# shreyasren/GPU-DualGradient-MPC

Hardware: AMD Instinct MI355X
Metric: GPAD iterations/s (instance-iterations, solve to eps=1e-4) (higher is better)
Workload: dtype f32

## Files before the change

### gpu-dualgradient-mpc_amd/csrc/gpad_compact.hip

```cpp
#include <hip/hip_runtime.h>

#include "gpad_internal.h"

namespace gpad {

constexpr int kSortMax = 8192;
constexpr int kSortBins = 4096;
__device__ __forceinline__ int block_scan_1024(int* part, int tid, int v) {
    const int lane = tid & 63, w = tid >> 6;
    int x = v;
#pragma unroll
    for (int off = 1; off < 64; off <<= 1) {
        const int y = __shfl_up(x, off);
        if (lane >= off) x += y;
    }
    if (lane == 63) part[w] = x;
    __syncthreads();
    int wb = 0;
    for (int i = 0; i < w; ++i) wb += part[i];
    __syncthreads();
    return wb + x - v;
}

constexpr int kCompactMaxPanels = 8192;
constexpr int kCompactU = 8;
__global__ __launch_bounds__(1024) void phase_compact_kernel(const int* __restrict__ seg_cnt,
                                                             const int* __restrict__ seg_idx, const int* count_prev,
                                                             int batch, int fin_prev, int* idx, int* count_out,
                                                             const int* pred, int fin_cur) {
    __shared__ int hist[kSortBins];
    __shared__ int ids[kSortMax];
    __shared__ int part[1024];
    __shared__ int pbase[kCompactMaxPanels];
    __shared__ int pcnt[kCompactMaxPanels];
    __shared__ int total_l;
    const int tid = threadIdx.x;
    const int pmax = (batch + 15) / 16;
    const int per = (pmax + 1023) / 1024;
    const int p0 = tid * per < pmax ? tid * per : pmax, p1 = p0 + per < pmax ? p0 + per : pmax;
    constexpr int kPer = 8;
    int cl[kPer];
#pragma unroll
    for (int u = 0; u < kPer; ++u) cl[u] = (per <= kPer && p0 + u < p1) ? seg_cnt[p0 + u] : 0;
    const int prev = count_prev ? *count_prev : batch;
    if (count_prev && prev <= fin_prev) {
        if (tid == 0) *count_out = 0;
        return;
    }
    const int panels = (prev + 15) / 16;
    const bool lds_bases = panels <= kCompactMaxPanels;
    const int q1 = p1 < panels ? p1 : panels;
    int sum = 0;
    if (per <= kPer) {
#pragma unroll
        for (int u = 0; u < kPer; ++u) {
            if (p0 + u < q1) {
                if (lds_bases) pcnt[p0 + u] = cl[u];
                sum += cl[u];
            }
        }
    } else {
        for (int p = p0; p < q1; ++p) {
            const int c = seg_cnt[p];
            if (lds_bases) pcnt[p] = c;
            sum += c;
        }
    }
    int base = block_scan_1024(part, tid, sum);
    if (tid == 1023) total_l = base + sum;
    if (lds_bases) {
        for (int p = p0; p < q1; ++p) {
            const int c = pcnt[p];
            pbase[p] = c ? base : -1;
            base += c;
        }
    }
    __syncthreads();
    const int count = total_l;
    const bool sort = pred && count > 1 && count <= fin_cur && count <= kSortMax;
    int* dst = sort ? ids : idx;
    if (lds_bases) {
        for (int i0 = tid; i0 < 16 * panels; i0 += 1024 * kCompactU) {
            int v[kCompactU], at[kCompactU];
#pragma unroll
            for (int u = 0; u < kCompactU; ++u) {
                const int i = i0 + 1024 * u;
                at[u] = -1;
                v[u] = 0;
                if (i < 16 * panels) {
                    const int p = i >> 4, r = i & 15, b = pbase[p];
                    if (b >= 0 && r < pcnt[p]) {
                        at[u] = b + r;
                        v[u] = seg_idx[i];
                    }
                }
            }
#pragma unroll
            for (int u = 0; u < kCompactU; ++u)
                if (at[u] >= 0) dst[at[u]] = v[u];
        }
    } else {
        for (int p = p0; p < q1; ++p) {
            const int c = seg_cnt[p];
            for (int r = 0; r < c; ++r) dst[base + r] = seg_idx[16 * p + r];
            base += c;
        }
    }
    if (tid == 0) *count_out = count;
    if (!sort) return;
    __syncthreads();
    int bn[kSortMax / 1024];
#pragma unroll
    for (int u = 0; u < kSortMax / 1024; ++u) {
        const int i = tid + 1024 * u;
        bn[u] = 0;
        if (i < count) {
            const int q = pred[ids[i]];
            const int k = q < 0 ? 0 : (q >= kSortBins ? kSortBins - 1 : q);
            bn[u] = kSortBins - 1 - k;
        }
    }
    for (int i = tid; i < kSortBins; i += 1024) hist[i] = 0;
    __syncthreads();
#pragma unroll
    for (int u = 0; u < kSortMax / 1024; ++u)
        if (tid + 1024 * u < count) atomicAdd(&hist[bn[u]], 1);
    __syncthreads();
    int local[4], hs = 0;
#pragma unroll
    for (int q = 0; q < 4; ++q) {
        local[q] = hs;
        hs += hist[4 * tid + q];
    }
    const int hb = block_scan_1024(part, tid, hs);
#pragma unroll
    for (int q = 0; q < 4; ++q) hist[4 * tid + q] = hb + local[q];
    __syncthreads();
#pragma unroll
    for (int u = 0; u < kSortMax / 1024; ++u) {
        const int i = tid + 1024 * u;
        if (i < count) idx[atomicAdd(&hist[bn[u]], 1)] = ids[i];
    }
}

hipError_t launch_phase_compact(const int* seg_cnt, const int* seg_idx, const int* count_prev, int batch,
                                int fin_prev, int* idx_out, int* count_out, const int* pred, int fin_cur,
                                hipStream_t s) {
    hipLaunchKernelGGL(phase_compact_kernel, dim3(1), dim3(1024), 0, s, seg_cnt, seg_idx, count_prev, batch,
                       fin_prev, idx_out, count_out, pred, fin_cur);
    return hipGetLastError();
}

}
```

### gpu-dualgradient-mpc_amd/csrc/gpad_host.cpp

```cpp
#include <algorithm>
#include <cmath>
#include <memory>

#include "gpad_host.h"

static thread_local std::string g_last_error;

int gpad::set_last_error(int code, const std::string& msg) {
    g_last_error = msg;
    return code;
}

int reset_status(gpad_handle_t h, double tol, double floor_scale) {
    const bool fresh = h->status.p == nullptr;
    int rc = h->status.ensure(sizeof(RunStatus));
    if (rc) return rc;
    if (fresh) HIP_TRY(hipMemsetAsync(h->status.p, 0, sizeof(RunStatus), h->stream));
    h->last_tol = tol;
    h->last_floor_scale = floor_scale;
    h->failed_run = false;
    return GPAD_OK;
}

static int fetch_status(gpad_handle_t h, RunStatus* rs, bool maxima = false) {
// ... 130 lines not shown
}

const char* gpad_last_error(void) { return g_last_error.c_str(); }

int gpad_create(gpad_handle_t* out, int device, void* stream) {
    return gpad::abi_guard("gpad_create", [&]() -> int {
        if (!out) return fail(GPAD_ERR_INVALID, "gpad_create: null handle pointer");
        *out = nullptr;
        int count = 0;
        const hipError_t e = hipGetDeviceCount(&count);
        if (e != hipSuccess) return fail(GPAD_ERR_NO_DEVICE, hip_detail("gpad_create: hipGetDeviceCount", e));
        if (count <= 0) return fail(GPAD_ERR_NO_DEVICE, "gpad_create: hipGetDeviceCount reported 0 devices");
        if (device < 0 || device >= count)
            return fail(GPAD_ERR_INVALID, "gpad_create: bad device index " + std::to_string(device) + " (" +
                                              std::to_string(count) + " visible)");
        HIP_TRY(hipSetDevice(device));
        auto h = std::make_unique<gpad_handle_s>();
        h->device = device;
        h->stream = static_cast<hipStream_t>(stream);
        {
            hipDeviceProp_t prop;
            if (hipGetDeviceProperties(&prop, device) == hipSuccess && prop.multiProcessorCount > 0)
                h->num_cus = prop.multiProcessorCount;
        }
        HIP_TRY(hipEventCreate(&h->ev0));
        HIP_TRY(hipEventCreate(&h->ev1));
        *out = h.release();
        return GPAD_OK;
    });
}

int gpad_destroy(gpad_handle_t h) {
    return gpad::abi_guard("gpad_destroy", [&]() -> int {
        if (!h) return GPAD_OK;
        (void)hipSetDevice(h->device);
        (void)hipStreamSynchronize(h->stream);
        end_classes(h);
        h->MGt.release();
        h->GLt.release();
        h->GLx.release();
        h->Hq.release();
        h->frows.release();
        h->frag64.release();
        h->hfrag64.release();
        h->q64.release();
        h->p64_order.release();
        h->frag.release();
        h->stage.release();
        h->theta.release();
        h->beta.release();
        h->work.release();
        h->counters.release();
        h->pwork.release();
        h->lipwork.release();
        h->status.release();
        h->own_plant.release();
        h->state.release();
        if (h->ev0) (void)hipEventDestroy(h->ev0);
        if (h->ev1) (void)hipEventDestroy(h->ev1);
        if (h->plan_ev) (void)hipEventDestroy(h->plan_ev);
        if (h->plan_pin) (void)hipHostFree(h->plan_pin);
        delete h;
        return GPAD_OK;
    });
}

int gpad_set_stream(gpad_handle_t h, void* stream) {
    return gpad::abi_guard("gpad_set_stream", [&]() -> int {
        if (!h) return fail(GPAD_ERR_INVALID, "gpad_set_stream: null handle");
        HIP_TRY(hipSetDevice(h->device));
        HIP_TRY(hipStreamSynchronize(h->stream));
        h->stream = static_cast<hipStream_t>(stream);
        if (h->cls) return gpad::classes_set_stream(h->cls, h->stream);
        return GPAD_OK;
    });
}

int gpad_set_option(gpad_handle_t h, int option, int value) {
    return gpad::abi_guard("gpad_set_option", [&]() -> int {
        if (!h) return fail(GPAD_ERR_INVALID, "gpad_set_option: null handle");
        const int rc = set_own_option(h, option, value);
        if (rc || !h->cls) return rc;
        HIP_TRY(hipSetDevice(h->device));
        return gpad::classes_set_option(h->cls, option, value);
    });
}

int gpad_sync(gpad_handle_t h) {
    return gpad::abi_guard("gpad_sync", [&]() -> int {
        if (!h) return fail(GPAD_ERR_INVALID, "gpad_sync: null handle");
        HIP_TRY(hipSetDevice(h->device));
        if (h->cls) return gpad::classes_sync(h->cls);
        RunStatus& rs = h->h_status;
        int rc = fetch_status(h, &rs);
        if (rc) return rc;
        HIP_TRY(hipStreamSynchronize(h->stream));
        return status_error(h, rs);
    });
}

int gpad_accumulate_iterations(gpad_handle_t h, long long* acc) {
    return gpad::abi_guard("gpad_accumulate_iterations", [&]() -> int {
        if (!h || !acc) return fail(GPAD_ERR_INVALID, "gpad_accumulate_iterations: null argument");
        if (h->cls) {
            HIP_TRY(hipSetDevice(h->device));
            return gpad::classes_accumulate(h->cls, acc);
// ... 187 lines not shown
```

### gpu-dualgradient-mpc_amd/csrc/gpad_host.h

```cpp
#pragma once

#include <hip/hip_runtime.h>

#include <cstddef>
#include <string>
#include <vector>

#include "../../include/gpad.h"
#include "gpad_abi.h"
#include "gpad_classes.h"
#include "gpad_internal.h"

inline int fail(int code, const std::string& msg) { return gpad::set_last_error(code, msg); }

inline std::string hip_detail(const std::string& what, hipError_t e) {
    return what + ": " + hipGetErrorName(e) + " (code " + std::to_string((int)e) + "): " + hipGetErrorString(e);
}

#define HIP_TRY(expr)                                                                        \
    do {                                                                                     \
        hipError_t _e = (expr);                                                              \
        if (_e != hipSuccess) {                                                              \
            return fail(_e == hipErrorOutOfMemory ? GPAD_ERR_NOMEM : GPAD_ERR_HIP,           \
                        hip_detail(#expr, _e));                                              \
// ... 48 lines not shown
    {GPAD_OPT_FLAT_WAVES, &gpad::Tuning::flat_waves, 0, 16, false},
    {GPAD_OPT_FLAT_A_LDS, &gpad::Tuning::flat_a_lds, 0, 1, false},
    {GPAD_OPT_DEBUG_DROP_HANDOFF, &gpad::Tuning::debug_drop_handoff, 0, 1, false},
    {GPAD_OPT_P64_RELAY, &gpad::Tuning::p64_no_relay, 0, 1, true},
    {GPAD_OPT_P64_REFILL, &gpad::Tuning::p64_no_refill, 0, 1, true},
    {GPAD_OPT_LOOP_ASYNC, &gpad::Tuning::loop_async, 0, 1, false},
    {GPAD_OPT_LOOP_PANEL, &gpad::Tuning::loop_panel, 0, 1, false},
};

struct RunStatus {
    int err;
    int pad;
    double part[gpad::kAbsmaxMaxBlocks];
    double acc[gpad::kAbsmaxMaxBlocks];
};

struct gpad_handle_s {
    int device = 0;
    hipStream_t stream = nullptr;
    bool ready = false;
    bool flat = false;
    int n_u = 0;
    gpad_dims_t dims{};
    double L = 1.0;
    bool scaled = false;
    int ldn = 0, ldm = 0;
    DevBuf MGt, GLt, frag, stage;
    bool frag_ok = false;
    bool keep_stage = false;
    std::vector<unsigned char> shadow;
    gpad_dims_t shadow_dims{};
    double shadow_L = 0.0;
    bool shadow_ok = false;
    DevBuf GLx;
    DevBuf Hq;
    bool hess_ok = false;
    double zbound = 0.0;
    DevBuf frows;
    DevBuf frag64;
    bool frag64_ok = false;
    int frag64_tiles = 0;
    DevBuf hfrag64;
    DevBuf q64;
    DevBuf p64_order;
    std::vector<int> p64_order_host;
    int p64_order_batch = 0;
    bool p64_order_dirty = false;
    bool last_p64 = false;
    bool hfrag64_ok = false;
    int frag_tiles = 0;
    DevBuf theta, beta;
    int sched_len = 0, sched_kind = -1, sched_dtype = -1;
    DevBuf work, counters, pwork;
    DevBuf lipwork;
    std::vector<int> h_counts;
    DevBuf status;
    RunStatus h_status;
    double last_tol = 0.0;
    double last_floor_scale = 0.0;
    hipEvent_t ev0 = nullptr, ev1 = nullptr;
    int last_kernel = 0, last_batch = 0, last_steps = 1;
    bool last_phased = false;
    int last_N = 0;
    gpad::PanelPlan plan;
    unsigned long long plan_key = 0;
    gpad::PanelPlan prior;
    bool last_prior = false;
    gpad::PanelPlan last_phases;
    int flat_vpred = 0;
    int* plan_pin = nullptr;
    size_t plan_pin_cap = 0;
    hipEvent_t plan_ev = nullptr;
    bool plan_pending = false;
    int plan_pending_N = 0, plan_pending_batch = 0;
    bool plan_pending_p64 = false;
    gpad::PlantStore own_plant;
    const gpad::PlantStore* plant = &own_plant;
    int plant_first = 0;
    bool plant_all = true;
    DevBuf state;
    int num_cus = 256;
    bool timed = false;
    gpad::Tuning tune;
    gpad::ClassBinding* cls = nullptr;
    const gpad::ClassLoop* cloop = nullptr;
    bool failed_run = false;
};

int reset_status(gpad_handle_t h, double tol, double floor_scale);
int collect_stats(gpad_handle_t h, gpad_stats_t* st);
void end_classes(gpad_handle_t h);
int no_classes(const char* fn);

int validate_dims(const gpad_dims_t* d);
void unbind_problem(gpad_handle_t h);
int ensure_schedule(gpad_handle_t h, int N, const void* theta_in, const void* beta_in);

void attach_plant(gpad_handle_t h, const gpad::PlantStore* store, int first, bool all);
bool loop_panel_shape(gpad_handle_t h, int N, double tol, int nxa);

void update_plan(gpad_handle_t h, const int* counts, int batch, int N);
void build_p64_order(gpad_handle_t h, const int* counts, int batch);
template <typename T>
void fill_solve_args(gpad_handle_t h, int N, double tol, gpad::SolveArgs<T>* a);
template <typename T>
int launch_solve(gpad_handle_t h, T* dz, T* dy, const T* dM, const T* dg, int N, double tol, bool scaled_vec,
// ... 2 lines not shown
```

### gpu-dualgradient-mpc_amd/csrc/gpad_internal.h

```cpp
#pragma once

#include <hip/hip_runtime.h>

#include <cstdint>
#include <string>

namespace gpad {

int set_last_error(int code, const std::string& msg);

struct ClassBinding;

struct Tuning {
    int phase_len = 0;
    int finish_thresh = -1;
    int plan = 1;
    int phased = 1;
    int lpt = 1;
    int panel_max_grid = 0;
    int duo_max_grid = 0;
    int flat_panel_min = -1;
    int flat_panels = 0;
    int flat_waves = 0;
    int flat_a_lds = 1;
// ... 26 lines not shown
}

template <typename T>
struct SolveArgs {
    const T* MGt;
    const T* GLt;
    long long strideA;
    long long strideB;
    const void* frag;
    int frag_tiles;
    const T* gP;
    const T* g;
    long long ld_gP, ld_g;
    double gscale;
    T* z;
    T* y;
    int n, m, ldn, ldm;
    int batch, N, check_every;
    double tol, L;
    double tol_gap;
    const T* theta;
    const T* beta;
    int* iters;
    int* conv;
    int num_cus;
    void* pwork;
    int v_begin, v_end;
    int v_pred;
    const int* idx_in;
    const int* count_in;
    int* idx_out;
    int* count_out;
    int* seg_cnt;
    int* seg_idx;
    double* gmax_part;
    int* zero_w;
    int zero_n;
    float* wc;
    float* uc;
    int fin_thresh;
    int* qctr;
    const int* pred;
    int n_u;
    int flat_staged;
    const int* order;
    const struct PanelPlan* plan;
    struct PanelPlan* used;
    const Tuning* tune;
    const T* Hq;
    long long strideHq;
    const void* hfrag64;
    int* err;
    int debug;
};

struct FarkasArgs;
template <typename T>
hipError_t launch_stream(const SolveArgs<T>& a, hipStream_t s, const FarkasArgs* fk = nullptr);
hipError_t launch_resident(const SolveArgs<float>& a, hipStream_t s, bool* supported, const FarkasArgs* fk = nullptr);
hipError_t launch_duo(const SolveArgs<float>& a, int grid, hipStream_t s);
bool resident_supported(int n, int m);
constexpr int kLoopMaxState = 64;
struct LoopArgs {
    SolveArgs<float> s;
    const float* PM;
    const float* M0;
    const float* Pg;
    const float* g0;
    const float* A;
    const float* B;
    const float* x_in;
    float* x_out;
    float* xs;
    float* us;
    double* gmax;
    int nx, nu, steps, warm;
    int per_plant;
    int ns;
    const float* S;
    int cls_K;
    const int* cls_off;
    const int* cls_start;
};
bool loop_supported(int n, int m, int nx, int nu);
int loop_blocks_per_cu(const LoopArgs& a, bool farkas = false);
hipError_t launch_loop(const LoopArgs& a, int grid, hipStream_t s, const FarkasArgs* fk = nullptr);
bool loop_panel_supported(int n, int m, int nx, int nu);
int loop_panel_grid(int n, int m, int batch, int num_cus, const Tuning* t);
hipError_t launch_loop_panel(const LoopArgs& a, int grid, hipStream_t s, const FarkasArgs* fk = nullptr);
bool panel64_supported(int n, int m);
int panel64_tiles(int n, int m);
size_t panel64_frag_bytes(int n, int m);
hipError_t launch_pack_panel64(const double* src, int rows, int cols, double scale, int T, void* dst, hipStream_t s);
hipError_t launch_panel64(const SolveArgs<double>& a, hipStream_t s);

typedef const __attribute__((address_space(4))) SolveArgs<float> KernArgs;
__device__ __forceinline__ KernArgs& kargs() {
    KernArgs* p = (KernArgs*)__builtin_amdgcn_kernarg_segment_ptr();
    asm volatile("" : "+s"(p));
    return *p;
}

template <class Args>
__device__ __forceinline__ void list_survivors(const Args& a, int P, bool park, int inst, int lane,
                                               int j) {
    const unsigned long long lv = __ballot(park && j == 0);
// ... 120 lines not shown
```

### gpu-dualgradient-mpc_amd/csrc/gpad_pairs.hip

```cpp
#include <hip/hip_runtime.h>

#include "gpad_internal.h"
#include "gpad_panel.h"

namespace gpad {

#ifdef GPAD_STAMP
#ifndef GPAD_STAMP_V0
#define GPAD_STAMP_V0 101
#endif
#ifndef GPAD_STAMP_PHASE_V
#define GPAD_STAMP_PHASE_V 100
#endif
constexpr int kStampV0 = GPAD_STAMP_V0, kStampIts = 4, kStampPts = 8;
__device__ unsigned long long g_stamps[16][kStampIts][kStampPts];
#define GPAD_STAMP_AT(P)                                      \
    do {                                                      \
        __builtin_amdgcn_sched_barrier(0);                    \
        stv[P] = __builtin_amdgcn_s_memtime();                \
        __builtin_amdgcn_sched_barrier(0);                    \
    } while (0)
#define GPAD_STAMP_FLUSH()                                                                  \
    do {                                                                                    \
        if (blockIdx.x == 0 && v >= kStampV0 && v < kStampV0 + kStampIts && lane == 0)      \
            for (int q_ = 0; q_ < kStampPts; ++q_) g_stamps[threadIdx.x >> 6][v - kStampV0][q_] = stv[q_]; \
    } while (0)
#define GPAD_STAMP_DECL unsigned long long stv[kStampPts] = {0, 0, 0, 0, 0, 0, 0, 0};
constexpr int kStampPhaseV = GPAD_STAMP_PHASE_V, kStampPhasePts = 10;
__device__ unsigned long long g_pstamps[16][kStampPhasePts];
#define GPAD_PSTAMP(P)                                                                              \
    do {                                                                                            \
        __builtin_amdgcn_sched_barrier(0);                                                          \
        if (blockIdx.x == 0 && a.v_begin == kStampPhaseV && (threadIdx.x & 63) == 0)               \
            g_pstamps[threadIdx.x >> 6][P] = __builtin_amdgcn_s_memtime();                          \
        __builtin_amdgcn_sched_barrier(0);                                                          \
    } while (0)
#define GPAD_STAMP_PTR(P) (&stv[P])
#define GPAD_PSTAMP_END(P)                  \
    do {                                    \
        if (v >= a.v_end) GPAD_PSTAMP(P);   \
    } while (0)
#else
#define GPAD_PSTAMP_END(P) \
    do {                   \
    } while (0)
#define GPAD_STAMP_AT(P) \
    do {                 \
    } while (0)
#define GPAD_STAMP_FLUSH() \
    do {                   \
    } while (0)
#define GPAD_STAMP_DECL
#define GPAD_STAMP_PTR(P) nullptr
#define GPAD_PSTAMP(P) \
    do {               \
    } while (0)
#endif

}

#include "gpad_pairs.h"

namespace gpad {

template <int T, int KQ, bool DROP = false>
__global__ __launch_bounds__(1024) void gpad_panel2_kernel(SolveArgs<float> a) {
    static_assert(T > 8 && T <= 16, "panel pairs need 8 < T <= 16");
    constexpr int D = 2 * T - 16;
    __shared__ Panel2Lds<T> L;
    const int count = a.count_in ? __builtin_amdgcn_readfirstlane(*a.count_in) : a.batch;
    if (a.count_in && count <= a.fin_thresh) return;
    const int panels = (count + 15) / 16;
    const bool pair = panels > (int)gridDim.x;
    const int w0 = __builtin_amdgcn_readfirstlane(threadIdx.x >> 6);
    const int w = pair ? ((w0 >> 1) == 4 ? w0 + 4 : ((w0 >> 1) == 6 ? w0 - 4 : w0)) : 15 - w0;
    const int items = pair ? (panels + 1) / 2 : panels;
    const bool ho = Handoff<T>::on && (KQ > 0 || (16 * (T - 1) < a.n && 16 * (T - 1) < a.m &&
                                                  (a.m + 15) / 16 == T && (a.n + 15) / 16 == T));
    if (threadIdx.x < 6) L.hflag[threadIdx.x] = 0;
    if (threadIdx.x == 0) {
        L.herr = 0;
        L.hdrop = DROP && blockIdx.x == 0;
    }
    if (threadIdx.x < 16) L.gred[threadIdx.x] = 0.0f;
    if (blockIdx.x == 0) {
        if (a.zero_w)
            for (int i = threadIdx.x; i < a.zero_n; i += blockDim.x) a.zero_w[i] = 0;
        if (a.gmax_part && a.v_begin == 0)
            for (int i = gridDim.x + threadIdx.x; i < kAbsmaxMaxBlocks; i += blockDim.x) a.gmax_part[i] = 0.0;
    }
    __syncthreads();
    if constexpr (Handoff<T>::on) {
        using H = Handoff<T>;
        if (pair) {
            if (w < D) panel2_run<T, 2, 0, 0, 0, false, KQ, DROP>(a, L, w, 0, true, items, count);
            else if (ho && w >= 14)
                panel2_run<T, 1, 1, 0, H::S, false, KQ, DROP>(a, L, T - 1, w & 1, true, items, count, HoSlots{-1, w & 1});
            else if (ho && w >= 12)
                panel2_run<T, 1, 2, H::S, 0, false, KQ, DROP>(a, L, T - 2, w & 1, true, items, count, HoSlots{w & 1, -1});
            else panel2_run<T, 1, 0, 0, 0, false, KQ, DROP>(a, L, D + ((w - D) >> 1), (w - D) & 1, true, items, count);
        } else {
            if constexpr (!H::relay) {
                if (w < T) panel2_run<T, 1, 0, 0, 0, false, 0, DROP>(a, L, w, 0, false, items, count);
                else panel2_run<T, 0, 0, 0, 0, false, 0, DROP>(a, L, 0, 0, false, items, count);
            } else if (ho && w == T - 1) panel2_run<T, 1, 2, H::R2, 0, true, 0, DROP>(a, L, w, 0, false, items, count, HoSlots{1, -1});
            else if (ho && w == T)
                panel2_run<T, 0, 3, 0, H::R1, true, 0, DROP>(a, L, T - 1, 0, false, items, count, HoSlots{-1, 0});
            else if (ho && w == T + 1)
                panel2_run<T, 0, 3, H::R1, H::R2, true, 0, DROP>(a, L, T - 1, 0, false, items, count, HoSlots{0, 1});
            else if (w < T)
                panel2_run<T, 1, 0, 0, 0, false, 0, DROP>(a, L, w, 0, false, items, count);
            else panel2_run<T, 0, 0, 0, 0, false, 0, DROP>(a, L, 0, 0, false, items, count);
        }
    } else if (pair) {
        if (w < D) panel2_run<T, 2, 0, 0, 0, false, KQ, DROP>(a, L, w, 0, true, items, count);
        else panel2_run<T, 1, 0, 0, 0, false, KQ, DROP>(a, L, D + ((w - D) >> 1), (w - D) & 1, true, items, count);
    } else {
        if (w < T) panel2_run<T, 1, 0, 0, 0, false, 0, DROP>(a, L, w, 0, false, items, count);
        else panel2_run<T, 0, 0, 0, 0, false, 0, DROP>(a, L, 0, 0, false, items, count);
    }
    if (Handoff<T>::on || a.gmax_part) {
        __syncthreads();
        if (Handoff<T>::on && threadIdx.x == 0 && L.herr) atomicOr(a.err, kDevErrHandoff);
        if (a.gmax_part && threadIdx.x == 0) {
            float g = 0.0f;
            for (int i = 0; i < 16; ++i) g = absmax_nan(g, L.gred[i]);
            a.gmax_part[blockIdx.x] = a.v_begin == 0 ? (double)g : absmax_nan(a.gmax_part[blockIdx.x], (double)g);
        }
    }
}

template <int T>
static void launch_pairs_t(const SolveArgs<float>& a, int grid, hipStream_t s) {
    if constexpr (T == 13) {
        const int kq1 = (a.m - 16 * (T - 1) + 3) / 4, kq2 = (a.n - 16 * (T - 1) + 3) / 4;
        const bool full = panel_handoff_shape(T, a.n, a.m) && kq1 == kq2;
        if (a.debug & kDebugDropHandoff) {
            if (full && kq1 == 2) hipLaunchKernelGGL((gpad_panel2_kernel<T, 2, true>), dim3(grid), dim3(1024), 0, s, a);
            else hipLaunchKernelGGL((gpad_panel2_kernel<T, 0, true>), dim3(grid), dim3(1024), 0, s, a);
            return;
        }
        if (full && kq1 == 1) { hipLaunchKernelGGL((gpad_panel2_kernel<T, 1>), dim3(grid), dim3(1024), 0, s, a); return; }
        if (full && kq1 == 2) { hipLaunchKernelGGL((gpad_panel2_kernel<T, 2>), dim3(grid), dim3(1024), 0, s, a); return; }
        if (full && kq1 == 3) { hipLaunchKernelGGL((gpad_panel2_kernel<T, 3>), dim3(grid), dim3(1024), 0, s, a); return; }
        if (full && kq1 == 4) { hipLaunchKernelGGL((gpad_panel2_kernel<T, 4>), dim3(grid), dim3(1024), 0, s, a); return; }
    }
    hipLaunchKernelGGL((gpad_panel2_kernel<T, 0>), dim3(grid), dim3(1024), 0, s, a);
}

hipError_t launch_panel_pairs(int T, const SolveArgs<float>& a, int grid, hipStream_t s) {
    switch (T) {
        case 9: launch_pairs_t<9>(a, grid, s); break;
        case 10: launch_pairs_t<10>(a, grid, s); break;
        case 11: launch_pairs_t<11>(a, grid, s); break;
        case 12: launch_pairs_t<12>(a, grid, s); break;
        case 13: launch_pairs_t<13>(a, grid, s); break;
        case 14: launch_pairs_t<14>(a, grid, s); break;
        case 15: launch_pairs_t<15>(a, grid, s); break;
        case 16: launch_pairs_t<16>(a, grid, s); break;
        default: return hipErrorInvalidValue;
    }
    return hipGetLastError();
}

#ifdef GPAD_STAMP
hipError_t read_stamps(unsigned long long* out, size_t bytes) {
    size_t b0 = bytes > sizeof(g_stamps) ? sizeof(g_stamps) : bytes;
    hipError_t e = hipMemcpyFromSymbol(out, HIP_SYMBOL(g_stamps), b0, 0, hipMemcpyDeviceToHost);
    if (e != hipSuccess || bytes <= sizeof(g_stamps)) return e;
    size_t b1 = bytes - sizeof(g_stamps);
    if (b1 > sizeof(g_pstamps)) b1 = sizeof(g_pstamps);
    return hipMemcpyFromSymbol(out + sizeof(g_stamps) / 8, HIP_SYMBOL(g_pstamps), b1, 0, hipMemcpyDeviceToHost);
}
#endif

}
```

### gpu-dualgradient-mpc_amd/csrc/gpad_phases.cpp

```cpp
#include <hip/hip_runtime.h>

#include <vector>

#include "gpad_farkas.h"
#include "gpad_internal.h"
#include "gpad_panel.h"

namespace gpad {

int panel_phase_len(int check_every, const Tuning* t) {
    int len = 4 * check_every;
    if (t && t->phase_len > 0) len = t->phase_len;
    return ((len + check_every - 1) / check_every) * check_every;
}

int panel_fin_thresh(int n, int m, int num_cus, const Tuning* t) {
    int f = resident_supported(n, m) ? 2 * num_cus : 0;
    if (t && t->finish_thresh >= 0 && f) f = t->finish_thresh;
    return f;
}

namespace {
struct PlanModel {
    int T, n, m, num_cus, grid;
// ... 161 lines not shown
    return w;
}
}

size_t panel_work_bytes(int m, int batch) { return phase_work(nullptr, m, batch).bytes; }

static hipError_t launch_panel_phase(int T, const SolveArgs<float>& a, int grid, hipStream_t s,
                                     const FarkasArgs* fk) {
    if (fk) return launch_panel_single(T, a, grid, s, fk);
    if (T == 0) {
        (void)launch_bigpanel(a, grid, s);
        return hipGetLastError();
    }
    return T > 8 ? launch_panel_pairs(T, a, grid, s) : launch_panel_single(T, a, grid, s);
}

static hipError_t launch_panel_phases(int T, SolveArgs<float> a, hipStream_t s, const FarkasArgs* fk) {
    const int panels = (a.batch + 15) / 16;
    const int resident = fk && T > 8 ? 2 * a.num_cus : panel_resident_grid(T, a.num_cus);
    int grid = panels < resident ? panels : resident;
    const Tuning tn = a.tune ? *a.tune : Tuning{};
    if (tn.panel_max_grid > 0 && tn.panel_max_grid < grid) grid = tn.panel_max_grid;
    const bool phased = a.tol > 0.0 && a.pwork != nullptr && tn.phased;
    a.fin_thresh = phased && !fk ? panel_fin_thresh(a.n, a.m, a.num_cus, &tn) : 0;
    if (!phased) {
        a.v_begin = 0;
        a.v_end = a.N;
        a.idx_in = nullptr;
        a.count_in = nullptr;
        return launch_panel_phase(T, a, grid, s, fk);
    }
    const PhaseWork w = phase_work(a.pwork, a.m, a.batch);
    a.wc = w.wc;
    a.uc = w.uc;
    a.seg_idx = w.seg_idx;
    a.seg_cnt = w.seg_cnt;
    a.idx_out = nullptr;
    a.count_out = nullptr;
    hipError_t e = hipSuccess;
    if (T > 8 && !fk) {
        a.zero_w = w.counts;
        a.zero_n = 2 * kPanelMaxPhases;
    } else if ((e = hipMemsetAsync(w.counts, 0, sizeof(int) * 2 * kPanelMaxPhases, s)) != hipSuccess) {
        return e;
    }
    const int len = panel_phase_len(a.check_every, &tn);
    const PanelPlan* plan = (a.plan && a.plan->nph > 0 && a.plan->N == a.N) ? a.plan : nullptr;
    if (a.used) {
        a.used->nph = 0;
        a.used->N = a.N;
        a.used->cost_us = plan ? plan->cost_us : 0.0;
    }
    const int fin_default = a.fin_thresh;
    int fin_prev = 0;
    int v0 = 0;
    for (int ph = 0; v0 < a.N; ++ph) {
        int plen = len;
        if (ph >= 10 && tn.phase_len <= 0) plen = len << (ph - 9 < 20 ? ph - 9 : 20);
        a.fin_thresh = fin_default;
        if (plan && ph < plan->nph) {
            plen = plan->ends[ph] - v0;
            if (ph && fin_default) a.fin_thresh = plan->fins[ph];
        }
        if (plen < 1) plen = len;
        if (ph >= kPanelMaxPhases - 1) plen = a.N;
        const int v1 = (a.N - v0 <= plen) ? a.N : v0 + plen;
        a.v_begin = v0;
        a.v_end = v1;
        a.idx_in = ph ? w.idx0 : nullptr;
        a.count_in = ph ? w.counts + ph - 1 : nullptr;
        if (ph) {
            e = launch_phase_compact(a.seg_cnt, a.seg_idx, ph >= 2 ? w.counts + ph - 2 : nullptr, a.batch, fin_prev,
                                     w.idx0, w.counts + ph - 1, (a.pred && tn.lpt) ? a.pred : nullptr, a.fin_thresh, s);
            if (e != hipSuccess) return e;
        }
        fin_prev = a.fin_thresh;
        if (a.used && ph < kPanelMaxPhases) {
            a.used->ends[ph] = v1;
            a.used->fins[ph] = ph ? a.fin_thresh : 0;
            a.used->nph = ph + 1;
        }
        if (ph && a.fin_thresh) {
            a.qctr = w.qctrs + ph;
            int g = a.fin_thresh < a.num_cus ? a.fin_thresh : a.num_cus;
            if (tn.duo_max_grid > 0 && tn.duo_max_grid < g) g = tn.duo_max_grid;
            if ((e = launch_duo(a, g, s)) != hipSuccess) return e;
        }
        if ((e = launch_panel_phase(T, a, grid, s, fk)) != hipSuccess) return e;
        a.zero_w = nullptr;
        v0 = v1;
    }
    return hipSuccess;
}

bool panel_folds_gmax(int n, int m) { return panel_tiles_for(n, m) > 8; }

hipError_t launch_panel(const SolveArgs<float>& a, hipStream_t s, bool* supported, const FarkasArgs* fk) {
    const int T = panel_tiles_for(a.n, a.m);
    if (fk && T < 1) {
        *supported = false;
        return hipSuccess;
    }
    *supported = a.frag != nullptr && a.strideA == 0 && a.strideB == 0 &&
                 (T ? a.frag_tiles == T
                    : bigpanel_supported(a.n, a.m) && a.frag_tiles == panel_tiles(a.n, a.m, a.batch));
    return *supported ? launch_panel_phases(T, a, s, fk) : hipSuccess;
}

hipError_t launch_flatpanel(const SolveArgs<float>& a0, hipStream_t s) {
    if (!flatpanel_supported(a0.n, a0.m, a0.n_u) || !a0.frag) return hipErrorInvalidValue;
    SolveArgs<float> a = a0;
    const Tuning tn = a.tune ? *a.tune : Tuning{};
    a.v_begin = 0;
    a.v_end = a.N;
    a.idx_in = nullptr;
    a.count_in = nullptr;
    const int panels = (a.batch + 15) / 16;
    const bool phased = a.tol > 0.0 && a.pwork != nullptr &&
                        (tn.phased == 2 || (tn.phased == 1 && panels >= 4 * a.num_cus));
    if (!phased) return launch_flatpanel_once(a, s);
    const PhaseWork w = phase_work(a.pwork, a.m, a.batch);
    a.wc = w.wc;
    a.uc = w.uc;
    hipError_t e = hipMemsetAsync(w.counts, 0, sizeof(int) * kPanelMaxPhases, s);
    if (e != hipSuccess) return e;
    int v0 = 0;
    for (int ph = 0; v0 < a.N; ++ph) {
        int plen = ph >= kPanelMaxPhases - 1 ? a.N : flat_phase_len(v0, a.check_every, &tn);
        if (a0.v_pred > 0 && v0 >= a0.v_pred) plen = a.N;
        const int v1 = (a.N - v0 <= plen) ? a.N : v0 + plen;
        a.v_begin = v0;
        a.v_end = v1;
        a.idx_in = ph ? ((ph & 1) ? w.idx0 : w.idx1) : nullptr;
        a.count_in = ph ? w.counts + ph - 1 : nullptr;
        a.idx_out = (ph & 1) ? w.idx1 : w.idx0;
        a.count_out = w.counts + ph;
        if ((e = launch_flatpanel_once(a, s)) != hipSuccess) return e;
        v0 = v1;
    }
// ... 5 lines not shown
```

### gpu-dualgradient-mpc_amd/csrc/gpad_run.cpp

```cpp
#include <algorithm>
#include <cmath>
#include <cstring>
#include <map>
#include <mutex>
#include <tuple>

#include "gpad_farkas.h"
#include "gpad_host.h"

using PlanShape = std::tuple<int, int, int, int, int, int, int>;
static std::mutex g_prior_mu;
static std::map<PlanShape, gpad::PanelPlan>& prior_plans() {
    static std::map<PlanShape, gpad::PanelPlan> m;
    return m;
}
static PlanShape plan_shape(gpad_handle_t h, int batch, int N) {
    return PlanShape{h->dims.n, h->dims.m, batch, h->dims.check_every, N, h->num_cus, h->tune.finish_thresh};
}
static void plan_prior_store(gpad_handle_t h, int batch, int N) {
    if (h->plan.nph <= 0) return;
    std::lock_guard<std::mutex> lk(g_prior_mu);
    auto& m = prior_plans();
    if (m.size() >= 64 && !m.count(plan_shape(h, batch, N))) m.clear();
    m[plan_shape(h, batch, N)] = h->plan;
// ... 163 lines not shown
                    if (int ro = h->p64_order.ensure(sizeof(int) * (size_t)batch)) return ro;
                    HIP_TRY(hipMemcpyAsync(h->p64_order.p, h->p64_order_host.data(), sizeof(int) * (size_t)batch,
                                           hipMemcpyHostToDevice, h->stream));
                    h->p64_order_dirty = false;
                }
                a.order = static_cast<const int*>(h->p64_order.p);
            }
            e = gpad::launch_panel64(a, h->stream);
            if (e != hipSuccess) return fail(GPAD_ERR_HIP, hip_detail("f64 panel", e));
            h->last_p64 = tol > 0.0;
            *kernel_out = GPAD_KERNEL_PANEL;
            return finish(GPAD_OK);
        }
    }
    if (a.Hq) {
        if (kernel != GPAD_KERNEL_AUTO && kernel != GPAD_KERNEL_STREAM)
            return fail(GPAD_ERR_UNSUPPORTED, "the value-function test (gpad_setup_hessian) runs on the stream kernel "
                                              "(f32) or the stream / f64 panel kernels (f64)");
        kernel = GPAD_KERNEL_STREAM;
    }
    if constexpr (sizeof(T) == sizeof(float)) {
        if (kernel == GPAD_KERNEL_STREAM && !h->flat) {
        } else if (h->flat) {
            a.n_u = h->n_u;
            const int fpm = h->tune.flat_panel_min >= 0 ? h->tune.flat_panel_min : (h->GLx.p ? 8 * h->num_cus : 0);
            if (h->frag_ok && (kernel == GPAD_KERNEL_PANEL || (kernel == GPAD_KERNEL_AUTO && batch >= fpm))) {
                if (tol > 0.0) {
                    int rc = h->pwork.ensure(gpad::panel_work_bytes(m, batch));
                    if (rc) return rc;
                    a.pwork = h->pwork.p;
                    a.v_pred = h->flat_vpred;
                }
                e = gpad::launch_flatpanel(a, h->stream);
                h->last_phased = a.pwork != nullptr;
            } else if (h->GLx.p && kernel != GPAD_KERNEL_STREAM) {
                a.GLt = (const T*)h->GLx.p;
                a.strideA = a.strideB = 0;
                e = gpad::launch_flat_resident(a, h->stream);
            } else {
                e = gpad::launch_flat(a, h->stream);
            }
            if (e != hipSuccess)
                return fail(e == hipErrorInvalidValue ? GPAD_ERR_UNSUPPORTED : GPAD_ERR_HIP,
                            std::string("flat kernel: ") + hipGetErrorString(e));
            *kernel_out = GPAD_KERNEL_FLAT;
            return finish(GPAD_OK);
        }
        const int panel_min = gpad::resident_supported(n, m) ? 4 * h->num_cus : 64;
        if (kernel == GPAD_KERNEL_PANEL || (kernel == GPAD_KERNEL_AUTO && d.shared && batch > panel_min)) {
            if (tol > 0.0 && h->frag_ok) {
                int rc = h->pwork.ensure(gpad::panel_work_bytes(m, batch));
                if (rc) return rc;
                a.pwork = h->pwork.p;
                a.plan = plan_for(h, batch, N);
                a.used = &h->last_phases;
                if (prev_phased && h->last_batch == batch && h->last_steps == 1) a.pred = iters;
            }
            e = gpad::launch_panel(a, h->stream, &ok);
            if (e != hipSuccess) return fail(GPAD_ERR_HIP, std::string("panel: ") + hipGetErrorString(e));
            if (ok) kernel = GPAD_KERNEL_PANEL;
            else if (kernel == GPAD_KERNEL_PANEL)
                return fail(GPAD_ERR_UNSUPPORTED, "panel kernel: needs shared f32 matrices");
            gmax_done = ok && gpad::panel_folds_gmax(n, m);
        }
        if (!ok && (kernel == GPAD_KERNEL_RESIDENT || kernel == GPAD_KERNEL_AUTO)) {
            e = gpad::launch_resident(a, h->stream, &ok);
            if (e != hipSuccess) return fail(GPAD_ERR_HIP, std::string("resident: ") + hipGetErrorString(e));
            if (ok) kernel = GPAD_KERNEL_RESIDENT;
            else if (kernel == GPAD_KERNEL_RESIDENT)
                return fail(GPAD_ERR_UNSUPPORTED, "resident kernel: needs n, m <= 208");
        }
    } else {
        if (kernel == GPAD_KERNEL_PANEL || kernel == GPAD_KERNEL_RESIDENT)
            return fail(GPAD_ERR_UNSUPPORTED, "f64: the resident kernel is f32 only; the f64 panels need shared "
                                              "matrices with n, m <= 256");
    }
    if (!ok) {
        kernel = GPAD_KERNEL_STREAM;
        e = gpad::launch_stream<T>(a, h->stream);
        if (e != hipSuccess)
            return fail(e == hipErrorInvalidValue ? GPAD_ERR_UNSUPPORTED : GPAD_ERR_HIP,
                        std::string("stream kernel: ") + hipGetErrorString(e) +
                            " (n+m beyond the LDS budget?)");
    }
    *kernel_out = kernel;
    h->last_phased = kernel == GPAD_KERNEL_PANEL && a.pwork != nullptr;
    return finish(GPAD_OK);
}
template int launch_solve<float>(gpad_handle_t, float*, float*, const float*, const float*, int, double, bool, int*,
                                 int*, int*);
template int launch_solve<double>(gpad_handle_t, double*, double*, const double*, const double*, int, double, bool,
                                  int*, int*, int*);

template <typename T>
static int run_typed(gpad_handle_t h, T* z, T* y, const T* M, const T* g, int N, double tol,
                     const void* theta_in, const void* beta_in, bool scaled_vec, gpad_stats_t* st) {
    const gpad_dims_t& d = h->dims;
    const int n = d.n, m = d.m, batch = d.batch;
    int rc = ensure_schedule(h, N, theta_in, beta_in);
    if (rc) return rc;
    if ((rc = h->counters.ensure(sizeof(int) * 2 * (size_t)batch))) return rc;
    T *dz = z, *dy = y;
    const T *dM = M, *dg = g;
    const size_t zb = sizeof(T) * (size_t)batch * n, yb = sizeof(T) * (size_t)batch * m;
    if (d.memory == GPAD_MEM_HOST) {
        if ((rc = h->work.ensure(2 * zb + 2 * yb))) return rc;
// ... 163 lines not shown
```

Before: 696.9 million.

## Fuse phase compaction into last-finishing panel workgroup via atomic ticket

The separate single-block compaction kernel launched between panel phases is folded into the panel-pair kernel. Each workgroup takes an atomic ticket at exit, and the last one runs the compaction for the next phase using LDS shared with the panel storage. This is meant to remove one kernel launch and a serialization gap per phase. In exchange, one workgroup's tail does serial work, and correctness depends on fences and on the ticket wrapping so it resets itself.

```diff
diff --git a/gpu-dualgradient-mpc_amd/csrc/gpad_compact.h b/gpu-dualgradient-mpc_amd/csrc/gpad_compact.h
--- /dev/null
+++ b/gpu-dualgradient-mpc_amd/csrc/gpad_compact.h
@@ -0,0 +1,153 @@
+#pragma once
+
+#include <hip/hip_runtime.h>
+
+namespace gpad {
+
+constexpr int kSortMax = 8192;
+constexpr int kSortBins = 4096;
+constexpr int kCompactMaxPanels = 8192;
+constexpr int kCompactU = 8;
+
+struct CompactLds {
+    int hist[kSortBins];
+    int ids[kSortMax];
+    int part[16];
+    int pbase[kCompactMaxPanels];
+    int pcnt[kCompactMaxPanels];
+    int total;
+};
+
+__device__ __forceinline__ int compact_ld(const int* p) {
+    return __hip_atomic_load(p, __ATOMIC_RELAXED, __HIP_MEMORY_SCOPE_AGENT);
+}
+
+__device__ __forceinline__ int block_scan_1024(int* part, int tid, int v) {
+    const int lane = tid & 63, w = tid >> 6;
+    int x = v;
+#pragma unroll
+    for (int off = 1; off < 64; off <<= 1) {
+        const int y = __shfl_up(x, off);
+        if (lane >= off) x += y;
+    }
+    if (lane == 63) part[w] = x;
+    __syncthreads();
+    int wb = 0;
+    for (int i = 0; i < w; ++i) wb += part[i];
+    __syncthreads();
+    return wb + x - v;
+}
+
+__device__ __forceinline__ void phase_compact(CompactLds& S, const int* seg_cnt, const int* seg_idx,
+                                              const int* count_prev, int batch, int fin_prev, int* idx,
+                                              int* count_out, const int* pred, int fin_cur) {
+    const int tid = threadIdx.x;
+    const int pmax = (batch + 15) / 16;
+    const int per = (pmax + 1023) / 1024;
+    const int p0 = tid * per < pmax ? tid * per : pmax, p1 = p0 + per < pmax ? p0 + per : pmax;
+    constexpr int kPer = 8;
+    int cl[kPer];
+#pragma unroll
+    for (int u = 0; u < kPer; ++u) cl[u] = (per <= kPer && p0 + u < p1) ? compact_ld(seg_cnt + p0 + u) : 0;
+    const int prev = count_prev ? *count_prev : batch;
+    if (count_prev && prev <= fin_prev) {
+        if (tid == 0) *count_out = 0;
+        return;
+    }
+    const int panels = (prev + 15) / 16;
+    const bool lds_bases = panels <= kCompactMaxPanels;
+    const int q1 = p1 < panels ? p1 : panels;
+    int sum = 0;
+    if (per <= kPer) {
+#pragma unroll
+        for (int u = 0; u < kPer; ++u) {
+            if (p0 + u < q1) {
+                if (lds_bases) S.pcnt[p0 + u] = cl[u];
+                sum += cl[u];
+            }
+        }
+    } else {
+        for (int p = p0; p < q1; ++p) {
+            const int c = compact_ld(seg_cnt + p);
+            if (lds_bases) S.pcnt[p] = c;
+            sum += c;
+        }
+    }
+    int base = block_scan_1024(S.part, tid, sum);
+    if (tid == 1023) S.total = base + sum;
+    if (lds_bases) {
+        for (int p = p0; p < q1; ++p) {
+            const int c = S.pcnt[p];
+            S.pbase[p] = c ? base : -1;
+            base += c;
+        }
+    }
+    __syncthreads();
+    const int count = S.total;
+    const bool sort = pred && count > 1 && count <= fin_cur && count <= kSortMax;
+    int* dst = sort ? S.ids : idx;
+    if (lds_bases) {
+        for (int i0 = tid; i0 < 16 * panels; i0 += 1024 * kCompactU) {
+            int v[kCompactU], at[kCompactU];
+#pragma unroll
+            for (int u = 0; u < kCompactU; ++u) {
+                const int i = i0 + 1024 * u;
+                at[u] = -1;
+                v[u] = 0;
+                if (i < 16 * panels) {
+                    const int p = i >> 4, r = i & 15, b = S.pbase[p];
+                    if (b >= 0 && r < S.pcnt[p]) {
+                        at[u] = b + r;
+                        v[u] = compact_ld(seg_idx + i);
+                    }
+                }
+            }
+#pragma unroll
+            for (int u = 0; u < kCompactU; ++u)
+                if (at[u] >= 0) dst[at[u]] = v[u];
+        }
+    } else {
+        for (int p = p0; p < q1; ++p) {
+            const int c = compact_ld(seg_cnt + p);
+            for (int r = 0; r < c; ++r) dst[base + r] = compact_ld(seg_idx + 16 * p + r);
+            base += c;
+        }
+    }
+    if (tid == 0) *count_out = count;
+    if (!sort) return;
+    __syncthreads();
+    int bn[kSortMax / 1024];
+#pragma unroll
+    for (int u = 0; u < kSortMax / 1024; ++u) {
+        const int i = tid + 1024 * u;
+        bn[u] = 0;
+        if (i < count) {
+            const int q = pred[S.ids[i]];
+            const int k = q < 0 ? 0 : (q >= kSortBins ? kSortBins - 1 : q);
+            bn[u] = kSortBins - 1 - k;
+        }
+    }
+    for (int i = tid; i < kSortBins; i += 1024) S.hist[i] = 0;
+    __syncthreads();
+#pragma unroll
+    for (int u = 0; u < kSortMax / 1024; ++u)
+        if (tid + 1024 * u < count) atomicAdd(&S.hist[bn[u]], 1);
+    __syncthreads();
+    int local[4], hs = 0;
+#pragma unroll
+    for (int q = 0; q < 4; ++q) {
+        local[q] = hs;
+        hs += S.hist[4 * tid + q];
+    }
+    const int hb = block_scan_1024(S.part, tid, hs);
+#pragma unroll
+    for (int q = 0; q < 4; ++q) S.hist[4 * tid + q] = hb + local[q];
+    __syncthreads();
+#pragma unroll
+    for (int u = 0; u < kSortMax / 1024; ++u) {
+        const int i = tid + 1024 * u;
+        if (i < count) idx[atomicAdd(&S.hist[bn[u]], 1)] = S.ids[i];
+    }
+}
+
+}
diff --git a/gpu-dualgradient-mpc_amd/csrc/gpad_compact.hip b/gpu-dualgradient-mpc_amd/csrc/gpad_compact.hip
--- a/gpu-dualgradient-mpc_amd/csrc/gpad_compact.hip
+++ b/gpu-dualgradient-mpc_amd/csrc/gpad_compact.hip
@@ -1,146 +1,15 @@
 #include <hip/hip_runtime.h>
 
+#include "gpad_compact.h"
 #include "gpad_internal.h"
 
 namespace gpad {
 
-constexpr int kSortMax = 8192;
-constexpr int kSortBins = 4096;
-__device__ __forceinline__ int block_scan_1024(int* part, int tid, int v) {
-    const int lane = tid & 63, w = tid >> 6;
-    int x = v;
-#pragma unroll
-    for (int off = 1; off < 64; off <<= 1) {
-        const int y = __shfl_up(x, off);
-        if (lane >= off) x += y;
-    }
-    if (lane == 63) part[w] = x;
-    __syncthreads();
-    int wb = 0;
-    for (int i = 0; i < w; ++i) wb += part[i];
-    __syncthreads();
-    return wb + x - v;
-}
-
-constexpr int kCompactMaxPanels = 8192;
-constexpr int kCompactU = 8;
-__global__ __launch_bounds__(1024) void phase_compact_kernel(const int* __restrict__ seg_cnt,
-                                                             const int* __restrict__ seg_idx, const int* count_prev,
-                                                             int batch, int fin_prev, int* idx, int* count_out,
-                                                             const int* pred, int fin_cur) {
-    __shared__ int hist[kSortBins];
-    __shared__ int ids[kSortMax];
-    __shared__ int part[1024];
-    __shared__ int pbase[kCompactMaxPanels];
-    __shared__ int pcnt[kCompactMaxPanels];
-    __shared__ int total_l;
-    const int tid = threadIdx.x;
-    const int pmax = (batch + 15) / 16;
-    const int per = (pmax + 1023) / 1024;
-    const int p0 = tid * per < pmax ? tid * per : pmax, p1 = p0 + per < pmax ? p0 + per : pmax;
-    constexpr int kPer = 8;
-    int cl[kPer];
-#pragma unroll
-    for (int u = 0; u < kPer; ++u) cl[u] = (per <= kPer && p0 + u < p1) ? seg_cnt[p0 + u] : 0;
-    const int prev = count_prev ? *count_prev : batch;
-    if (count_prev && prev <= fin_prev) {
-        if (tid == 0) *count_out = 0;
-        return;
-    }
-    const int panels = (prev + 15) / 16;
-    const bool lds_bases = panels <= kCompactMaxPanels;
-    const int q1 = p1 < panels ? p1 : panels;
-    int sum = 0;
-    if (per <= kPer) {
-#pragma unroll
-        for (int u = 0; u < kPer; ++u) {
-            if (p0 + u < q1) {
-                if (lds_bases) pcnt[p0 + u] = cl[u];
-                sum += cl[u];
-            }
-        }
-    } else {
-        for (int p = p0; p < q1; ++p) {
-            const int c = seg_cnt[p];
-            if (lds_bases) pcnt[p] = c;
-            sum += c;
-        }
-    }
-    int base = block_scan_1024(part, tid, sum);
-    if (tid == 1023) total_l = base + sum;
-    if (lds_bases) {
-        for (int p = p0; p < q1; ++p) {
-            const int c = pcnt[p];
-            pbase[p] = c ? base : -1;
-            base += c;
-        }
-    }
-    __syncthreads();
-    const int count = total_l;
-    const bool sort = pred && count > 1 && count <= fin_cur && count <= kSortMax;
-    int* dst = sort ? ids : idx;
-    if (lds_bases) {
-        for (int i0 = tid; i0 < 16 * panels; i0 += 1024 * kCompactU) {
-            int v[kCompactU], at[kCompactU];
-#pragma unroll
-            for (int u = 0; u < kCompactU; ++u) {
-                const int i = i0 + 1024 * u;
-                at[u] = -1;
-                v[u] = 0;
-                if (i < 16 * panels) {
-                    const int p = i >> 4, r = i & 15, b = pbase[p];
-                    if (b >= 0 && r < pcnt[p]) {
-                        at[u] = b + r;
-                        v[u] = seg_idx[i];
-                    }
-                }
-            }
-#pragma unroll
-            for (int u = 0; u < kCompactU; ++u)
-                if (at[u] >= 0) dst[at[u]] = v[u];
-        }
-    } else {
-        for (int p = p0; p < q1; ++p) {
-            const int c = seg_cnt[p];
-            for (int r = 0; r < c; ++r) dst[base + r] = seg_idx[16 * p + r];
-            base += c;
-        }
-    }
-    if (tid == 0) *count_out = count;
-    if (!sort) return;
-    __syncthreads();
-    int bn[kSortMax / 1024];
-#pragma unroll
-    for (int u = 0; u < kSortMax / 1024; ++u) {
-        const int i = tid + 1024 * u;
-        bn[u] = 0;
-        if (i < count) {
-            const int q = pred[ids[i]];
-            const int k = q < 0 ? 0 : (q >= kSortBins ? kSortBins - 1 : q);
-            bn[u] = kSortBins - 1 - k;
-        }
-    }
-    for (int i = tid; i < kSortBins; i += 1024) hist[i] = 0;
-    __syncthreads();
-#pragma unroll
-    for (int u = 0; u < kSortMax / 1024; ++u)
-        if (tid + 1024 * u < count) atomicAdd(&hist[bn[u]], 1);
-    __syncthreads();
-    int local[4], hs = 0;
-#pragma unroll
-    for (int q = 0; q < 4; ++q) {
-        local[q] = hs;
-        hs += hist[4 * tid + q];
-    }
-    const int hb = block_scan_1024(part, tid, hs);
-#pragma unroll
-    for (int q = 0; q < 4; ++q) hist[4 * tid + q] = hb + local[q];
-    __syncthreads();
-#pragma unroll
-    for (int u = 0; u < kSortMax / 1024; ++u) {
-        const int i = tid + 1024 * u;
-        if (i < count) idx[atomicAdd(&hist[bn[u]], 1)] = ids[i];
-    }
+__global__ __launch_bounds__(1024) void phase_compact_kernel(const int* seg_cnt, const int* seg_idx,
+                                                             const int* count_prev, int batch, int fin_prev, int* idx,
+                                                             int* count_out, const int* pred, int fin_cur) {
+    __shared__ CompactLds S;
+    phase_compact(S, seg_cnt, seg_idx, count_prev, batch, fin_prev, idx, count_out, pred, fin_cur);
 }
 
 hipError_t launch_phase_compact(const int* seg_cnt, const int* seg_idx, const int* count_prev, int batch,
diff --git a/gpu-dualgradient-mpc_amd/csrc/gpad_host.cpp b/gpu-dualgradient-mpc_amd/csrc/gpad_host.cpp
--- a/gpu-dualgradient-mpc_amd/csrc/gpad_host.cpp
+++ b/gpu-dualgradient-mpc_amd/csrc/gpad_host.cpp
@@ -206,6 +206,7 @@
         h->work.release();
         h->counters.release();
         h->pwork.release();
+        h->ptick.release();
         h->lipwork.release();
         h->status.release();
         h->own_plant.release();
diff --git a/gpu-dualgradient-mpc_amd/csrc/gpad_host.h b/gpu-dualgradient-mpc_amd/csrc/gpad_host.h
--- a/gpu-dualgradient-mpc_amd/csrc/gpad_host.h
+++ b/gpu-dualgradient-mpc_amd/csrc/gpad_host.h
@@ -124,6 +124,7 @@
     DevBuf theta, beta;
     int sched_len = 0, sched_kind = -1, sched_dtype = -1;
     DevBuf work, counters, pwork;
+    DevBuf ptick;
     DevBuf lipwork;
     std::vector<int> h_counts;
     DevBuf status;
diff --git a/gpu-dualgradient-mpc_amd/csrc/gpad_internal.h b/gpu-dualgradient-mpc_amd/csrc/gpad_internal.h
--- a/gpu-dualgradient-mpc_amd/csrc/gpad_internal.h
+++ b/gpu-dualgradient-mpc_amd/csrc/gpad_internal.h
@@ -102,6 +102,12 @@
     const void* hfrag64;
     int* err;
     int debug;
+    int* tickets;
+    int* cmp_ticket;
+    int* cmp_idx;
+    int* cmp_count;
+    const int* cmp_pred;
+    int cmp_fin;
 };
 
 struct FarkasArgs;
diff --git a/gpu-dualgradient-mpc_amd/csrc/gpad_pairs.hip b/gpu-dualgradient-mpc_amd/csrc/gpad_pairs.hip
--- a/gpu-dualgradient-mpc_amd/csrc/gpad_pairs.hip
+++ b/gpu-dualgradient-mpc_amd/csrc/gpad_pairs.hip
@@ -1,5 +1,6 @@
 #include <hip/hip_runtime.h>
 
+#include "gpad_compact.h"
 #include "gpad_internal.h"
 #include "gpad_panel.h"
 
@@ -67,9 +68,15 @@
 __global__ __launch_bounds__(1024) void gpad_panel2_kernel(SolveArgs<float> a) {
     static_assert(T > 8 && T <= 16, "panel pairs need 8 < T <= 16");
     constexpr int D = 2 * T - 16;
-    __shared__ Panel2Lds<T> L;
+    constexpr size_t kLdsBytes = sizeof(Panel2Lds<T>) > sizeof(CompactLds) ? sizeof(Panel2Lds<T>) : sizeof(CompactLds);
+    __shared__ __attribute__((aligned(16))) unsigned char lds[kLdsBytes];
+    __shared__ int last_wg;
+    Panel2Lds<T>& L = *reinterpret_cast<Panel2Lds<T>*>(lds);
     const int count = a.count_in ? __builtin_amdgcn_readfirstlane(*a.count_in) : a.batch;
-    if (a.count_in && count <= a.fin_thresh) return;
+    if (a.count_in && count <= a.fin_thresh) {
+        if (a.cmp_ticket && blockIdx.x == 0 && threadIdx.x == 0) *a.cmp_count = 0;
+        return;
+    }
     const int panels = (count + 15) / 16;
     const bool pair = panels > (int)gridDim.x;
     const int w0 = __builtin_amdgcn_readfirstlane(threadIdx.x >> 6);
@@ -128,6 +135,19 @@
             a.gmax_part[blockIdx.x] = a.v_begin == 0 ? (double)g : absmax_nan(a.gmax_part[blockIdx.x], (double)g);
         }
     }
+    KernArgs& A = kargs();
+    if (A.cmp_ticket) {
+        __syncthreads();
+        if (threadIdx.x == 0) {
+            __builtin_amdgcn_fence(__ATOMIC_RELEASE, "agent");
+            last_wg = atomicInc(reinterpret_cast<unsigned*>(A.cmp_ticket), gridDim.x - 1) == gridDim.x - 1;
+            __builtin_amdgcn_fence(__ATOMIC_ACQUIRE, "agent");
+        }
+        __syncthreads();
+        if (!last_wg) return;
+        phase_compact(*reinterpret_cast<CompactLds*>(lds), A.seg_cnt, A.seg_idx, A.count_in, A.batch, A.fin_thresh,
+                      A.cmp_idx, A.cmp_count, A.cmp_pred, A.cmp_fin);
+    }
 }
 
 template <int T>
diff --git a/gpu-dualgradient-mpc_amd/csrc/gpad_phases.cpp b/gpu-dualgradient-mpc_amd/csrc/gpad_phases.cpp
--- a/gpu-dualgradient-mpc_amd/csrc/gpad_phases.cpp
+++ b/gpu-dualgradient-mpc_amd/csrc/gpad_phases.cpp
@@ -237,26 +237,32 @@
         a.used->cost_us = plan ? plan->cost_us : 0.0;
     }
     const int fin_default = a.fin_thresh;
+    auto schedule = [&](int ph, int v0, int* fin) -> int {
+        int plen = len;
+        if (ph >= 10 && tn.phase_len <= 0) plen = len << (ph - 9 < 20 ? ph - 9 : 20);
+        *fin = fin_default;
+        if (plan && ph < plan->nph) {
+            plen = plan->ends[ph] - v0;
+            if (ph && fin_default) *fin = plan->fins[ph];
+        }
+        if (plen < 1) plen = len;
+        if (ph >= kPanelMaxPhases - 1) plen = a.N;
+        return (a.N - v0 <= plen) ? a.N : v0 + plen;
+    };
+    const bool fused = T > 8 && !fk && a.tickets != nullptr;
+    const int* const lpt_pred = (a.pred && tn.lpt) ? a.pred : nullptr;
     int fin_prev = 0;
     int v0 = 0;
     for (int ph = 0; v0 < a.N; ++ph) {
-        int plen = len;
-        if (ph >= 10 && tn.phase_len <= 0) plen = len << (ph - 9 < 20 ? ph - 9 : 20);
-        a.fin_thresh = fin_default;
-        if (plan && ph < plan->nph) {
-            plen = plan->ends[ph] - v0;
-            if (ph && fin_default) a.fin_thresh = plan->fins[ph];
-        }
-        if (plen < 1) plen = len;
-        if (ph >= kPanelMaxPhases - 1) plen = a.N;
-        const int v1 = (a.N - v0 <= plen) ? a.N : v0 + plen;
+        const int v1 = schedule(ph, v0, &a.fin_thresh);
         a.v_begin = v0;
         a.v_end = v1;
         a.idx_in = ph ? w.idx0 : nullptr;
         a.count_in = ph ? w.counts + ph - 1 : nullptr;
-        if (ph) {
+        a.cmp_ticket = nullptr;
+        if (ph && !fused) {
             e = launch_phase_compact(a.seg_cnt, a.seg_idx, ph >= 2 ? w.counts + ph - 2 : nullptr, a.batch, fin_prev,
-                                     w.idx0, w.counts + ph - 1, (a.pred && tn.lpt) ? a.pred : nullptr, a.fin_thresh, s);
+                                     w.idx0, w.counts + ph - 1, lpt_pred, a.fin_thresh, s);
             if (e != hipSuccess) return e;
         }
         fin_prev = a.fin_thresh;
@@ -270,6 +276,13 @@
             int g = a.fin_thresh < a.num_cus ? a.fin_thresh : a.num_cus;
             if (tn.duo_max_grid > 0 && tn.duo_max_grid < g) g = tn.duo_max_grid;
             if ((e = launch_duo(a, g, s)) != hipSuccess) return e;
+        }
+        if (fused && v1 < a.N) {
+            a.cmp_ticket = a.tickets + ph;
+            a.cmp_idx = w.idx0;
+            a.cmp_count = w.counts + ph;
+            a.cmp_pred = lpt_pred;
+            (void)schedule(ph + 1, v1, &a.cmp_fin);
         }
         if ((e = launch_panel_phase(T, a, grid, s, fk)) != hipSuccess) return e;
         a.zero_w = nullptr;
diff --git a/gpu-dualgradient-mpc_amd/csrc/gpad_run.cpp b/gpu-dualgradient-mpc_amd/csrc/gpad_run.cpp
--- a/gpu-dualgradient-mpc_amd/csrc/gpad_run.cpp
+++ b/gpu-dualgradient-mpc_amd/csrc/gpad_run.cpp
@@ -239,6 +239,13 @@
                 int rc = h->pwork.ensure(gpad::panel_work_bytes(m, batch));
                 if (rc) return rc;
                 a.pwork = h->pwork.p;
+                if (!h->ptick.p) {
+                    if ((rc = h->ptick.ensure(sizeof(int) * gpad::kPanelMaxPhases))) return rc;
+                    const hipError_t ez = hipMemsetAsync(h->ptick.p, 0, sizeof(int) * gpad::kPanelMaxPhases, h->stream);
+                    if (ez != hipSuccess) h->ptick.release();
+                    HIP_TRY(ez);
+                }
+                a.tickets = static_cast<int*>(h->ptick.p);
                 a.plan = plan_for(h, batch, N);
                 a.used = &h->last_phases;
                 if (prev_phased && h->last_batch == batch && h->last_steps == 1) a.pred = iters;
```

Result: no change. 694.0 million (-0.4%).
